# ChenKaiXuSan/Skiing_Analysis_PyTorch

Measured on AMD Instinct MI355X. Metric: 3D-pose frames/sec, 8-view 518px clips, higher is better.
Workload: dtype f16

## Files before the change

skiing_analysis_pytorch_amd/csrc/common.h:

```cpp
#pragma once
#include <hip/hip_runtime.h>
#include <stdint.h>
#include <stdio.h>
#include <atomic>
#include <string>

#include "../../include/skimi.h"

namespace skimi {

void set_error(const char* fmt, ...);

#define SKIMI_CHECK_ARG(cond, ...)            \
    do {                                      \
        if (!(cond)) {                        \
            ::skimi::set_error(__VA_ARGS__);  \
            return SKIMI_ERR_ARG;             \
        }                                     \
    } while (0)

#define SKIMI_HIP(call)                                                                  \
    do {                                                                                 \
        hipError_t e_ = (call);                                                          \
        if (e_ != hipSuccess) {                                                          \
// ... 58 lines not shown
typedef __attribute__((ext_vector_type(8))) _Float16 f16x8;
template <bool F16>
__device__ __forceinline__ f32x16 mfma_32x32x16(bf16x8 a, bf16x8 b, f32x16 c) {
    if constexpr (F16)
        return __builtin_amdgcn_mfma_f32_32x32x16_f16(__builtin_bit_cast(f16x8, a), __builtin_bit_cast(f16x8, b), c, 0, 0, 0);
    else
        return __builtin_amdgcn_mfma_f32_32x32x16_bf16(a, b, c, 0, 0, 0);
}
template <bool F16>
__device__ __forceinline__ f32x4 mfma_16x16x32(bf16x8 a, bf16x8 b, f32x4 c) {
    if constexpr (F16)
        return __builtin_amdgcn_mfma_f32_16x16x32_f16(__builtin_bit_cast(f16x8, a), __builtin_bit_cast(f16x8, b), c, 0, 0, 0);
    else
        return __builtin_amdgcn_mfma_f32_16x16x32_bf16(a, b, c, 0, 0, 0);
}
__device__ __forceinline__ unsigned mx_scale_byte(float amax) {
    if (!(amax > 0.f)) return 0u;
    const float t = amax * (1.0f / 448.0f);
    const unsigned u = __float_as_uint(t);
    const int e = (int)((u >> 23) & 0xFF) - 127 + ((u & 0x7FFFFF) ? 1 : 0);
    return (unsigned)min(max(e + 127, 1), 254);
}
__device__ __forceinline__ float mx_inv_scale(unsigned sb) { return sb ? __uint_as_float((unsigned)(254 - (int)sb) << 23) : 0.f; }
__device__ __forceinline__ int mx_pack4(float a, float b, float c, float d, float inv) {
    int w = 0;
    w = __builtin_amdgcn_cvt_pk_fp8_f32(a * inv, b * inv, w, false);
    w = __builtin_amdgcn_cvt_pk_fp8_f32(c * inv, d * inv, w, true);
    return w;
}
__device__ __forceinline__ float max8(float v) {
// ... 22 lines not shown
```

skiing_analysis_pytorch_amd/csrc/gemm_x3dma.hip:

```cpp
#include <stdlib.h>

#include <algorithm>

#include "common.h"
#include "gemm_epilogue.h"

namespace skimi {

typedef __attribute__((address_space(3))) void lds_void;
typedef __attribute__((address_space(1))) const void gbl_void;

__global__ __launch_bounds__(256) void split_planes_kernel(const float* __restrict__ x, long ld, long rows, int C,
                                                           unsigned short* __restrict__ hi, unsigned short* __restrict__ lo) {
    const int C4 = C / 4;
    const long total = rows * C4;
    for (long i = (long)blockIdx.x * 256 + threadIdx.x; i < total; i += (long)gridDim.x * 256) {
        const long r = i / C4;
        const int c = (int)(i - r * C4) * 4;
        const float4 v = *reinterpret_cast<const float4*>(x + r * ld + c);
        const float f[4] = {v.x, v.y, v.z, v.w};
        bf16x4 h, l;
#pragma unroll
        for (int k = 0; k < 4; ++k) {
            const unsigned short hb = f2bf(f[k]);
// ... 55 lines not shown
    const char* w;
    const char* zero;
    long a_row_bytes;
    long w_row_bytes;
    long a_bias;
};

#define SKIMI_X3_BAR()                        \
    do {                                      \
        __builtin_amdgcn_sched_barrier(0);    \
        __builtin_amdgcn_s_barrier();         \
        __builtin_amdgcn_sched_barrier(0);    \
    } while (0)
#define SKIMI_X3_VMCNT(N) __builtin_amdgcn_s_waitcnt(0x0F70 | ((N) & 15) | (((N) >> 4) << 14))

template <int AMODE, int ABL = 0>
__global__ __launch_bounds__(256, 1) void gemm_x3w4_kernel(const GemmArgs p, const X3Rec pl) {
    constexpr int BM = 256, BN = 256, BK = 32, RB = 128, PIECE = 128 * RB, NSLOT = 10;
    extern __shared__ __attribute__((aligned(16))) char smem[];

    const int tid = threadIdx.x, lane = tid & 63;
    const int wave = __builtin_amdgcn_readfirstlane(tid >> 6);
    const int wr = wave >> 1, wc = wave & 1;
    const int l31 = lane & 31, lh = lane >> 5;

    int id;
    {
        const int nblk = p.ntm * p.ntn;
        const int bid = blockIdx.x;
        const int xcd = bid & 7;
        const int q = nblk >> 3, r = nblk & 7;
        id = (xcd < r ? xcd * (q + 1) : r * (q + 1) + (xcd - r) * q) + (bid >> 3);
// ... 22 lines not shown
                const int rem = m - img * ohw;
                const int oy = rem / p.OW;
                const int iy0 = oy * p.stride - p.pad, ix0 = (rem - oy * p.OW) * p.stride - p.pad;
                a_off[q][j] = (unsigned)((((long)img * p.cH + iy0) * p.cW + ix0) * pl.a_row_bytes + c * 16 + pl.a_bias);
                unsigned ok = 0;
                for (int ky = 0; ky < p.KH; ++ky)
                    for (int kx = 0; kx < p.KW; ++kx) {
                        const int iy = iy0 + ky * p.dil, ix = ix0 + kx * p.dil;
                        if (iy >= 0 && iy < p.cH && ix >= 0 && ix < p.cW) ok |= 1u << (ky * p.KW + kx);
                    }
                a_ok[q][j] = ok;
            }
            w_off[q][j] = (unsigned)((long)min(n0 + 128 * q + row, p.N - 1) * pl.w_row_bytes + c * 16);
        }
    int cur_tap = 0, cur_ky = 0, cur_kx = 0, cur_cs = 0;
    auto issue_a = [&](int kt, int slot0, int slot1) {
        const int tap = cur_tap, tap_dy = cur_ky * p.dil, tap_dx = cur_kx * p.dil;
        const int cs = AMODE == 0 ? kt : cur_cs;
        if (AMODE == 2) {
            ++cur_tap;
            if (++cur_kx == p.KW) { cur_kx = 0; ++cur_ky; }
            if (cur_tap == p.KH * p.KW) { cur_tap = 0; cur_ky = 0; ++cur_cs; }
        } else if (AMODE == 1) {
            if (++cur_cs == p.cC / 32) {
                cur_cs = 0;
                ++cur_tap;
                if (++cur_kx == p.KW) { cur_kx = 0; ++cur_ky; }
            }
        }
        if (ABL & 1) return;
        const long kbytes = ((long)tap_dy * p.cW + tap_dx) * pl.a_row_bytes + (long)cs * 128 - (AMODE != 0 ? pl.a_bias : 0);
        const char* base = pl.a + kbytes;
        const unsigned z = (unsigned)(pl.zero - base);
#pragma unroll
        for (int q = 0; q < 2; ++q) {
            char* dst = smem + (q == 0 ? slot0 : slot1) * PIECE + (4 * wave) * 8 * RB;
#pragma unroll
            for (int j = 0; j < 4; ++j) {
                const bool ok = AMODE == 0 || ((a_ok[q][j] >> tap) & 1u) != 0;
                const unsigned o = ok ? a_off[q][j] : z + ((lane & 7) << 4);
                __builtin_amdgcn_global_load_lds((gbl_void*)(base + (size_t)o), (lds_void*)(dst + j * 8 * RB), 16, 0, 0);
            }
        }
    };
    auto issue_w = [&](int kt, int slot0, int slot1) {
        if (ABL & 1) return;
        const char* base = pl.w + (long)kt * 128;
#pragma unroll
        for (int q = 0; q < 2; ++q) {
            char* dst = smem + (q == 0 ? slot0 : slot1) * PIECE + (4 * wave) * 8 * RB;
#pragma unroll
            for (int j = 0; j < 4; ++j)
                __builtin_amdgcn_global_load_lds((gbl_void*)(base + (size_t)w_off[q][j]), (lds_void*)(dst + j * 8 * RB), 16, 0, 0);
        }
    };
    auto slot = [&](int x) { return x >= NSLOT ? x - NSLOT : x; };

    const int t = lh ^ ((l31 >> 1) & 7);
    const int lane_off = l31 * RB;
    bf16x8 ah0[4], al0[4], wh0[4], wl0[4], ah1[4], al1[4], wh1[4], wl1[4];
    if (ABL & 2) {
#pragma unroll
        for (int i = 0; i < 4; ++i) {
            const bf16x8 c = {(short)lane, 1, 2, 3, 4, 5, 6, 7};
            ah0[i] = al0[i] = wh0[i] = wl0[i] = ah1[i] = al1[i] = wh1[i] = wl1[i] = c;
        }
    }
    auto read = [&](int sb, int s, bf16x8 (&ah)[4], bf16x8 (&al)[4], bf16x8 (&wh)[4], bf16x8 (&wl)[4]) {
        if (ABL & 2) return;
        const int x = ((2 * s) ^ t) << 4;
        const char* pa = smem + slot(sb + wr) * PIECE + lane_off;
        const char* pw = smem + slot(sb + 2 + wc) * PIECE + lane_off;
#pragma unroll
        for (int i = 0; i < 4; ++i) {
            ah[i] = *reinterpret_cast<const bf16x8*>(pa + i * 32 * RB + x);
            al[i] = *reinterpret_cast<const bf16x8*>(pa + i * 32 * RB + (x ^ 64));
        }
#pragma unroll
        for (int i = 0; i < 4; ++i) {
            wh[i] = *reinterpret_cast<const bf16x8*>(pw + i * 32 * RB + x);
            wl[i] = *reinterpret_cast<const bf16x8*>(pw + i * 32 * RB + (x ^ 64));
        }
    };

    f32x16 acc[4][4];
#pragma unroll
    for (int i = 0; i < 4; ++i)
#pragma unroll
        for (int j = 0; j < 4; ++j)
#pragma unroll
            for (int r = 0; r < 16; ++r) acc[i][j][r] = 0.f;
#define SKIMI_X3_MFMA(AH, AL, WH, WL)                                                                             \
    do {                                                                                                           \
        if (ABL & 4) break;                                                                                        \
        _Pragma("unroll") for (int j = 0; j < 4; ++j) _Pragma("unroll") for (int i = 0; i < 4; ++i)                \
            acc[i][j] = __builtin_amdgcn_mfma_f32_32x32x16_bf16(AL[i], WH[j], acc[i][j], 0, 0, 0);                 \
        _Pragma("unroll") for (int j = 0; j < 4; ++j) _Pragma("unroll") for (int i = 0; i < 4; ++i)                \
            acc[i][j] = __builtin_amdgcn_mfma_f32_32x32x16_bf16(AH[i], WL[j], acc[i][j], 0, 0, 0);                 \
        _Pragma("unroll") for (int j = 0; j < 4; ++j) _Pragma("unroll") for (int i = 0; i < 4; ++i)                \
            acc[i][j] = __builtin_amdgcn_mfma_f32_32x32x16_bf16(AH[i], WH[j], acc[i][j], 0, 0, 0);                 \
// ... 49 lines not shown
        SKIMI_X3_MFMA(ah1, al1, wh1, wl1);                                          \
        if (N1) SKIMI_X3_TAIL((N2 ? 8 : 0)); else __builtin_amdgcn_sched_barrier(0); \
        sb = nsb;                                                                   \
    } while (0)
    int kt = 0;
    for (; kt + 2 < nkt; ++kt) SKIMI_X3_KTILE(true, true);
    if (kt + 1 < nkt) {
        SKIMI_X3_KTILE(true, false);
        ++kt;
    }
    SKIMI_X3_KTILE(false, false);
#undef SKIMI_X3_KTILE
#undef SKIMI_X3_TAIL
#undef SKIMI_X3_HEAD
#undef SKIMI_X3_MFMA
    __builtin_amdgcn_s_waitcnt(0xC07F);
    SKIMI_X3_BAR();

    float* stg = reinterpret_cast<float*>(smem) + wave * (32 * 128);
    const int n = n0 + wc * 128 + 4 * (lane & 31);
    const bool relu_ok = (p.act == SKIMI_ACT_NONE || p.act == SKIMI_ACT_RELU) &&
                         (p.post_act == SKIMI_ACT_NONE || p.post_act == SKIMI_ACT_RELU);
    const bool fast = p.vec4 && p.store_mode == 0 && p.out_rpb == 0 && p.out_off == 0 && p.out2 == nullptr &&
                      p.out_dtype == SKIMI_F32 && p.gamma == nullptr && relu_ok && (p.resid != nullptr || p.resid2 == nullptr) &&
                      (p.resid == nullptr || p.resid_dtype == SKIMI_F32) &&
                      m0 + BM <= p.M && n0 + BN <= p.N;
    if (fast) {
        const float lo1 = p.act == SKIMI_ACT_RELU ? 0.f : -__builtin_inff();
        const float lo2 = p.post_act == SKIMI_ACT_RELU ? 0.f : -__builtin_inff();
        float4 bs = make_float4(0.f, 0.f, 0.f, 0.f);
        if (p.bias) bs = *reinterpret_cast<const float4*>(p.bias + n);
        const float* rs = reinterpret_cast<const float*>(p.resid);
        const float* rs2 = reinterpret_cast<const float*>(p.resid2);
        float* out = reinterpret_cast<float*>(p.out);
        const int rpb = p.resid_rpb > 0 ? p.resid_rpb : 0x7fffffff;
        auto res_row = [&](long m) {
            const int b = (int)m / rpb;
            return ((long)b * p.resid_bs + ((int)m - b * rpb) + p.resid_off) * p.ldr;
        };
#define SKIMI_X3_EPI_PASS(HAS_RES, HAS_OUT, HAS_REC)                                                                                 \
    _Pragma("unroll") for (int i = 0; i < 4; ++i) {                                                                \
        _Pragma("unroll") for (int j = 0; j < 4; ++j) _Pragma("unroll") for (int r = 0; r < 16; ++r)               \
            stg[((r & 3) + 8 * (r >> 2) + 4 * lh) * 128 + j * 32 + l31] = acc[i][j][r];                           \
        __builtin_amdgcn_fence(__ATOMIC_RELEASE, "wavefront");                                                     \
        __builtin_amdgcn_s_waitcnt(0xC07F);                                                                        \
        _Pragma("unroll") for (int half = 0; half < 2; ++half) {                                                   \
            const long mrow = m0 + wr * 128 + i * 32 + half * 16 + lh;                                             \
            float4 v[8], rr[8], r2[8];                                                                             \
            _Pragma("unroll") for (int it = 0; it < 8; ++it)                                                       \
                v[it] = *reinterpret_cast<const float4*>(&stg[(half * 16 + it * 2 + lh) * 128 + 4 * (lane & 31)]); \
            if (HAS_RES) _Pragma("unroll") for (int it = 0; it < 8; ++it)                                          \
                rr[it] = *reinterpret_cast<const float4*>(rs + res_row(mrow + it * 2) + n);                       \
            if (HAS_RES == 2) _Pragma("unroll") for (int it = 0; it < 8; ++it)                                     \
                r2[it] = *reinterpret_cast<const float4*>(rs2 + (mrow + it * 2) * p.ldr2 + n);                     \
            _Pragma("unroll") for (int it = 0; it < 8; ++it) {                                                     \
                float4 y = make_float4(fmaxf(v[it].x + bs.x, lo1), fmaxf(v[it].y + bs.y, lo1),                     \
                                       fmaxf(v[it].z + bs.z, lo1), fmaxf(v[it].w + bs.w, lo1));                    \
                if (HAS_RES) { y.x += rr[it].x; y.y += rr[it].y; y.z += rr[it].z; y.w += rr[it].w; }               \
                if (HAS_RES == 2) { y.x += r2[it].x; y.y += r2[it].y; y.z += r2[it].z; y.w += r2[it].w; }          \
                y = make_float4(fmaxf(y.x, lo2), fmaxf(y.y, lo2), fmaxf(y.z, lo2), fmaxf(y.w, lo2));               \
                if (HAS_OUT) *reinterpret_cast<float4*>(out + (mrow + it * 2) * p.ldo + n) = y;                    \
                if (HAS_REC) store_rec4(p, mrow + it * 2, n, y.x, y.y, y.z, y.w);                                  \
            }                                                                                                      \
        }                                                                                                          \
        __builtin_amdgcn_s_waitcnt(0xC07F);                                                                        \
// ... 4 lines not shown
            case 10: SKIMI_X3_EPI_PASS(2, true, false) break;
            case 9: SKIMI_X3_EPI_PASS(2, false, true) break;
            case 7: SKIMI_X3_EPI_PASS(1, true, true) break;
            case 6: SKIMI_X3_EPI_PASS(1, true, false) break;
            case 5: SKIMI_X3_EPI_PASS(1, false, true) break;
            case 3: SKIMI_X3_EPI_PASS(0, true, true) break;
            case 2: SKIMI_X3_EPI_PASS(0, true, false) break;
            case 1: SKIMI_X3_EPI_PASS(0, false, true) break;
            default: break;
        }
#undef SKIMI_X3_EPI_PASS
        return;
    }
#pragma unroll
    for (int i = 0; i < 4; ++i) {
#pragma unroll
        for (int j = 0; j < 4; ++j)
#pragma unroll
            for (int r = 0; r < 16; ++r) stg[((r & 3) + 8 * (r >> 2) + 4 * lh) * 128 + j * 32 + l31] = acc[i][j][r];
        __builtin_amdgcn_fence(__ATOMIC_RELEASE, "wavefront");
        __builtin_amdgcn_s_waitcnt(0xC07F);
#pragma unroll 1
        for (int it = 0; it < 16; ++it) {
            const int row_l = it * 2 + lh;
            const int m = m0 + wr * 128 + i * 32 + row_l;
            if (m >= p.M || n >= p.N) continue;
            const float4 v = *reinterpret_cast<const float4*>(&stg[row_l * 128 + 4 * (lane & 31)]);
            const RowMap rm = row_map(p, m);
            if (p.vec4) {
                store_four(p, rm, n, v);
            } else {
                store_one(p, rm, n, v.x);
                if (n + 1 < p.N) store_one(p, rm, n + 1, v.y);
                if (n + 2 < p.N) store_one(p, rm, n + 2, v.z);
                if (n + 3 < p.N) store_one(p, rm, n + 3, v.w);
            }
        }
        __builtin_amdgcn_s_waitcnt(0xC07F);
    }
}

template <int AMODE>
__global__ __launch_bounds__(256, 1) void gemm_x3w4n_kernel(const GemmArgs p, const X3Rec pl) {
    constexpr int BM = 256, BN = 128, BK = 32, RB = 128, PIECE = 128 * RB, NSLOT = 9;
    extern __shared__ __attribute__((aligned(16))) char smem[];

    const int tid = threadIdx.x, lane = tid & 63;
    const int wave = __builtin_amdgcn_readfirstlane(tid >> 6);
    const int wr = wave >> 1, wc = wave & 1;
    const int l31 = lane & 31, lh = lane >> 5;

    int id;
    {
        const int nblk = p.ntm * p.ntn;
        const int bid = blockIdx.x;
        const int xcd = bid & 7;
        const int q = nblk >> 3, r = nblk & 7;
// ... 24 lines not shown
                const int oy = rem / p.OW;
                const int iy0 = oy * p.stride - p.pad, ix0 = (rem - oy * p.OW) * p.stride - p.pad;
                a_off[q][j] = (unsigned)((((long)img * p.cH + iy0) * p.cW + ix0) * pl.a_row_bytes + c * 16 + pl.a_bias);
                unsigned ok = 0;
                for (int ky = 0; ky < p.KH; ++ky)
                    for (int kx = 0; kx < p.KW; ++kx) {
                        const int iy = iy0 + ky * p.dil, ix = ix0 + kx * p.dil;
                        if (iy >= 0 && iy < p.cH && ix >= 0 && ix < p.cW) ok |= 1u << (ky * p.KW + kx);
                    }
                a_ok[q][j] = ok;
            }
        }
        w_off[j] = (unsigned)((long)min(n0 + row, p.N - 1) * pl.w_row_bytes + c * 16);
    }
    int cur_tap = 0, cur_ky = 0, cur_kx = 0, cur_cs = 0;
    auto issue = [&](int kt, int s0, int s1, int s2) {
        const int tap = cur_tap, tap_dy = cur_ky * p.dil, tap_dx = cur_kx * p.dil;
        const int cs = AMODE == 0 ? kt : cur_cs;
        if (AMODE == 2) {
            ++cur_tap;
            if (++cur_kx == p.KW) { cur_kx = 0; ++cur_ky; }
            if (cur_tap == p.KH * p.KW) { cur_tap = 0; cur_ky = 0; ++cur_cs; }
        } else if (AMODE == 1) {
            if (++cur_cs == p.cC / 32) {
                cur_cs = 0;
                ++cur_tap;
                if (++cur_kx == p.KW) { cur_kx = 0; ++cur_ky; }
            }
        }
        const long kbytes = ((long)tap_dy * p.cW + tap_dx) * pl.a_row_bytes + (long)cs * 128 - (AMODE != 0 ? pl.a_bias : 0);
        const char* base = pl.a + kbytes;
        const unsigned z = (unsigned)(pl.zero - base);
#pragma unroll
        for (int q = 0; q < 2; ++q) {
            char* dst = smem + (q == 0 ? s0 : s1) * PIECE + (4 * wave) * 8 * RB;
#pragma unroll
            for (int j = 0; j < 4; ++j) {
                const bool ok = AMODE == 0 || ((a_ok[q][j] >> tap) & 1u) != 0;
                const unsigned o = ok ? a_off[q][j] : z + ((lane & 7) << 4);
                __builtin_amdgcn_global_load_lds((gbl_void*)(base + (size_t)o), (lds_void*)(dst + j * 8 * RB), 16, 0, 0);
            }
        }
        const char* wbase = pl.w + (long)kt * 128;
        char* dst = smem + s2 * PIECE + (4 * wave) * 8 * RB;
#pragma unroll
        for (int j = 0; j < 4; ++j)
            __builtin_amdgcn_global_load_lds((gbl_void*)(wbase + (size_t)w_off[j]), (lds_void*)(dst + j * 8 * RB), 16, 0, 0);
    };
    auto slot = [&](int x) { return x >= NSLOT ? x - NSLOT : x; };

    const int t = lh ^ ((l31 >> 1) & 7);
    const int fa_off = l31 * RB, fw_off = (wc * 64 + l31) * RB;
    bf16x8 ah0[4], al0[4], wh0[2], wl0[2], ah1[4], al1[4], wh1[2], wl1[2];
    auto read = [&](int sb, int s, bf16x8 (&ah)[4], bf16x8 (&al)[4], bf16x8 (&wh)[2], bf16x8 (&wl)[2]) {
        const int x = ((2 * s) ^ t) << 4;
        const char* pa = smem + slot(sb + wr) * PIECE + fa_off;
        const char* pw = smem + slot(sb + 2) * PIECE + fw_off;
#pragma unroll
        for (int i = 0; i < 4; ++i) {
            ah[i] = *reinterpret_cast<const bf16x8*>(pa + i * 32 * RB + x);
            al[i] = *reinterpret_cast<const bf16x8*>(pa + i * 32 * RB + (x ^ 64));
        }
#pragma unroll
        for (int i = 0; i < 2; ++i) {
            wh[i] = *reinterpret_cast<const bf16x8*>(pw + i * 32 * RB + x);
            wl[i] = *reinterpret_cast<const bf16x8*>(pw + i * 32 * RB + (x ^ 64));
        }
    };

    f32x16 acc[4][2];
#pragma unroll
    for (int i = 0; i < 4; ++i)
#pragma unroll
        for (int j = 0; j < 2; ++j)
#pragma unroll
            for (int r = 0; r < 16; ++r) acc[i][j][r] = 0.f;
#define SKIMI_X3N_MFMA(AH, AL, WH, WL)                                                                            \
    do {                                                                                                           \
        _Pragma("unroll") for (int j = 0; j < 2; ++j) _Pragma("unroll") for (int i = 0; i < 4; ++i)                \
            acc[i][j] = __builtin_amdgcn_mfma_f32_32x32x16_bf16(AL[i], WH[j], acc[i][j], 0, 0, 0);                 \
        _Pragma("unroll") for (int j = 0; j < 2; ++j) _Pragma("unroll") for (int i = 0; i < 4; ++i)                \
            acc[i][j] = __builtin_amdgcn_mfma_f32_32x32x16_bf16(AH[i], WL[j], acc[i][j], 0, 0, 0);                 \
        _Pragma("unroll") for (int j = 0; j < 2; ++j) _Pragma("unroll") for (int i = 0; i < 4; ++i)                \
            acc[i][j] = __builtin_amdgcn_mfma_f32_32x32x16_bf16(AH[i], WH[j], acc[i][j], 0, 0, 0);                 \
    } while (0)
// ... 46 lines not shown
    int kt = 0;
    for (; kt + 3 < nkt; ++kt) SKIMI_X3N_KTILE(true, true, true);
    if (kt + 2 < nkt) {
        SKIMI_X3N_KTILE(true, true, false);
        ++kt;
    }
    if (kt + 1 < nkt) {
        SKIMI_X3N_KTILE(true, false, false);
        ++kt;
    }
    SKIMI_X3N_KTILE(false, false, false);
#undef SKIMI_X3N_KTILE
#undef SKIMI_X3N_TAIL
#undef SKIMI_X3N_HEAD
#undef SKIMI_X3N_MFMA
    __builtin_amdgcn_s_waitcnt(0xC07F);
    SKIMI_X3_BAR();

    float* stg = reinterpret_cast<float*>(smem) + wave * (32 * 64);
    const int n = n0 + wc * 64 + 4 * (lane & 15);
    const bool relu_ok = (p.act == SKIMI_ACT_NONE || p.act == SKIMI_ACT_RELU) &&
                         (p.post_act == SKIMI_ACT_NONE || p.post_act == SKIMI_ACT_RELU);
    const bool fast = p.vec4 && p.store_mode == 0 && p.out_rpb == 0 && p.out_off == 0 && p.out2 == nullptr &&
                      p.out_dtype == SKIMI_F32 && p.gamma == nullptr && relu_ok && (p.resid != nullptr || p.resid2 == nullptr) &&
                      (p.resid == nullptr || p.resid_dtype == SKIMI_F32) &&
                      m0 + BM <= p.M && n0 + BN <= p.N;
    if (fast) {
        const float lo1 = p.act == SKIMI_ACT_RELU ? 0.f : -__builtin_inff();
        const float lo2 = p.post_act == SKIMI_ACT_RELU ? 0.f : -__builtin_inff();
        float4 bs = make_float4(0.f, 0.f, 0.f, 0.f);
        if (p.bias) bs = *reinterpret_cast<const float4*>(p.bias + n);
        const float* rs = reinterpret_cast<const float*>(p.resid);
        const float* rs2 = reinterpret_cast<const float*>(p.resid2);
        float* out = reinterpret_cast<float*>(p.out);
        const int rpb = p.resid_rpb > 0 ? p.resid_rpb : 0x7fffffff;
        auto res_row = [&](long m) {
            const int b = (int)m / rpb;
            return ((long)b * p.resid_bs + ((int)m - b * rpb) + p.resid_off) * p.ldr;
        };
#define SKIMI_X3N_EPI_PASS(HAS_RES, HAS_OUT, HAS_REC)                                                                                \
    _Pragma("unroll") for (int i = 0; i < 4; ++i) {                                                                \
        _Pragma("unroll") for (int j = 0; j < 2; ++j) _Pragma("unroll") for (int r = 0; r < 16; ++r)               \
            stg[((r & 3) + 8 * (r >> 2) + 4 * lh) * 64 + j * 32 + l31] = acc[i][j][r];                            \
        __builtin_amdgcn_fence(__ATOMIC_RELEASE, "wavefront");                                                     \
        __builtin_amdgcn_s_waitcnt(0xC07F);                                                                        \
        const long mrow = m0 + wr * 128 + i * 32 + (lane >> 4);                                                    \
        float4 v[8], rr[8], r2[8];                                                                                 \
        _Pragma("unroll") for (int it = 0; it < 8; ++it)                                                           \
            v[it] = *reinterpret_cast<const float4*>(&stg[(it * 4 + (lane >> 4)) * 64 + 4 * (lane & 15)]);         \
        if (HAS_RES) _Pragma("unroll") for (int it = 0; it < 8; ++it)                                              \
            rr[it] = *reinterpret_cast<const float4*>(rs + res_row(mrow + it * 4) + n);                           \
        if (HAS_RES == 2) _Pragma("unroll") for (int it = 0; it < 8; ++it)                                         \
            r2[it] = *reinterpret_cast<const float4*>(rs2 + (mrow + it * 4) * p.ldr2 + n);                         \
        _Pragma("unroll") for (int it = 0; it < 8; ++it) {                                                         \
            float4 y = make_float4(fmaxf(v[it].x + bs.x, lo1), fmaxf(v[it].y + bs.y, lo1),                         \
                                   fmaxf(v[it].z + bs.z, lo1), fmaxf(v[it].w + bs.w, lo1));                        \
            if (HAS_RES) { y.x += rr[it].x; y.y += rr[it].y; y.z += rr[it].z; y.w += rr[it].w; }                   \
            if (HAS_RES == 2) { y.x += r2[it].x; y.y += r2[it].y; y.z += r2[it].z; y.w += r2[it].w; }              \
            y = make_float4(fmaxf(y.x, lo2), fmaxf(y.y, lo2), fmaxf(y.z, lo2), fmaxf(y.w, lo2));                   \
            if (HAS_OUT) *reinterpret_cast<float4*>(out + (mrow + it * 4) * p.ldo + n) = y;                        \
            if (HAS_REC) store_rec4(p, mrow + it * 4, n, y.x, y.y, y.z, y.w);                                      \
        }                                                                                                          \
        __builtin_amdgcn_s_waitcnt(0xC07F);                                                                        \
    }
// ... 3 lines not shown
            case 10: SKIMI_X3N_EPI_PASS(2, true, false) break;
            case 9: SKIMI_X3N_EPI_PASS(2, false, true) break;
            case 7: SKIMI_X3N_EPI_PASS(1, true, true) break;
            case 6: SKIMI_X3N_EPI_PASS(1, true, false) break;
            case 5: SKIMI_X3N_EPI_PASS(1, false, true) break;
            case 3: SKIMI_X3N_EPI_PASS(0, true, true) break;
            case 2: SKIMI_X3N_EPI_PASS(0, true, false) break;
            case 1: SKIMI_X3N_EPI_PASS(0, false, true) break;
            default: break;
        }
#undef SKIMI_X3N_EPI_PASS
        return;
    }
#pragma unroll
    for (int i = 0; i < 4; ++i) {
#pragma unroll
        for (int j = 0; j < 2; ++j)
#pragma unroll
            for (int r = 0; r < 16; ++r) stg[((r & 3) + 8 * (r >> 2) + 4 * lh) * 64 + j * 32 + l31] = acc[i][j][r];
        __builtin_amdgcn_fence(__ATOMIC_RELEASE, "wavefront");
        __builtin_amdgcn_s_waitcnt(0xC07F);
#pragma unroll 1
        for (int it = 0; it < 8; ++it) {
            const int row_l = it * 4 + (lane >> 4);
            const int m = m0 + wr * 128 + i * 32 + row_l;
            if (m >= p.M || n >= p.N) continue;
            const float4 v = *reinterpret_cast<const float4*>(&stg[row_l * 64 + 4 * (lane & 15)]);
            const RowMap rm = row_map(p, m);
            if (p.vec4) {
                store_four(p, rm, n, v);
            } else {
                store_one(p, rm, n, v.x);
                if (n + 1 < p.N) store_one(p, rm, n + 1, v.y);
                if (n + 2 < p.N) store_one(p, rm, n + 2, v.z);
                if (n + 3 < p.N) store_one(p, rm, n + 3, v.w);
            }
        }
        __builtin_amdgcn_s_waitcnt(0xC07F);
    }
}

static long x3_rows_in(const skimi_gemm_desc* d) { return d->a_mode == 0 ? (long)d->M : (long)d->cN * d->cH * d->cW; }
// ... 17 lines not shown
        return false;
    }
    if (d->store_mode != 0 && d->store_mode != 1) return false;
    if (d->K % 4 != 0) return false;
    if (d->a_mode != 0 && (d->cC % 32 != 0 || d->KH * d->KW > 32)) return false;
    const long kp = ((long)d->K + 31) / 32 * 32;
    const long bias = d->a_mode == 0 ? 0 : ((long)d->pad * d->cW + d->pad) * x3_cp(d) * 4;
    if ((long)gemm_x3dma_scratch_bytes(d) + bias >= (1ll << 32) || (long)d->N * kp * 4 >= (1ll << 32)) return false;
    static const bool dyn = getenv("SKIMI_ENV_DYNAMIC") && atoi(getenv("SKIMI_ENV_DYNAMIC"));
    static long min_tiles = -1;
    if (min_tiles < 0 || dyn) min_tiles = getenv("SKIMI_X3_MIN_TILES") ? atol(getenv("SKIMI_X3_MIN_TILES")) : 160;
    const long tiles = cdiv(d->M, 256) * (d->N > 128 ? cdiv(d->N, 256) : 1);
    return d->M >= (min_tiles <= 1 ? 256 : 4096) && d->N >= 96 && tiles >= min_tiles;
}

template <int AMODE, int ABL = 0>
static int launch_x3w4(GemmArgs& a, const X3Rec& pl, hipStream_t st) {
    constexpr size_t lds = 10ull * 128 * 128;
    SKIMI_LDS_OPT_IN((gemm_x3w4_kernel<AMODE, ABL>), lds, "gemm_x3w4");
    a.ntm = (int)cdiv(a.M, 256);
    a.ntn = (int)cdiv(a.N, 256);
    a.splitk = 1;
    hipLaunchKernelGGL((gemm_x3w4_kernel<AMODE, ABL>), dim3(a.ntm * a.ntn), dim3(256), lds, st, a, pl);
    SKIMI_LAUNCH_CHECK();
    return SKIMI_OK;
}

template <int AMODE>
static int launch_x3w4n(GemmArgs& a, const X3Rec& pl, hipStream_t st) {
    constexpr size_t lds = 9ull * 128 * 128;
    SKIMI_LDS_OPT_IN(gemm_x3w4n_kernel<AMODE>, lds, "gemm_x3w4n");
    a.ntm = (int)cdiv(a.M, 256);
    a.ntn = (int)cdiv(a.N, 128);
    a.splitk = 1;
    hipLaunchKernelGGL(gemm_x3w4n_kernel<AMODE>, dim3(a.ntm * a.ntn), dim3(256), lds, st, a, pl);
    SKIMI_LAUNCH_CHECK();
    return SKIMI_OK;
}

int gemm_x3dma_launch(GemmArgs& a, const skimi_gemm_desc* d, hipStream_t st) {
    const long rows_in = x3_rows_in(d), cp = x3_cp(d);
    const int Cw = d->a_mode == 0 ? d->K : d->cC;
    char* rec = (char*)d->x3_scratch;
    char* zpage = rec + rows_in * cp * 4;
    if (d->a_dtype == SKIMI_BF16X3_REC) {
        rec = (char*)d->A;
        zpage = (char*)d->x3_scratch;
    } else {
        int rc = split_records_launch((const float*)d->A, d->lda, rows_in, Cw, rec, st, zpage);
        if (rc) return rc;
    }
    X3Rec pl;
    pl.a = rec;
    pl.w = (const char*)d->W_split;
    pl.zero = zpage;
    pl.a_row_bytes = cp * 4;
    pl.w_row_bytes = ((long)d->K + 31) / 32 * 32 * 4;
    pl.a_bias = d->a_mode == 0 ? 0 : ((long)d->pad * d->cW + d->pad) * pl.a_row_bytes;
    a.dbg = 0;
    set_gemm_path(d->N <= 128 ? SKIMI_GEMM_PATH_X3DMA_NARROW : SKIMI_GEMM_PATH_X3DMA_WIDE, 0, 0, 0, 1);
    if (d->N <= 128) {
        if (a.a_mode == 0) return launch_x3w4n<0>(a, pl, st);
        if (a.a_mode == 1) return launch_x3w4n<1>(a, pl, st);
        return launch_x3w4n<2>(a, pl, st);
    }
#ifdef SKIMI_ABLATIONS
    if (a.a_mode == 0) {
        static const int abl = getenv("SKIMI_X3_ABL") ? atoi(getenv("SKIMI_X3_ABL")) : 0;
        switch (abl) {
            case 1: return launch_x3w4<0, 1>(a, pl, st);
            case 2: return launch_x3w4<0, 2>(a, pl, st);
            case 3: return launch_x3w4<0, 3>(a, pl, st);
            case 5: return launch_x3w4<0, 5>(a, pl, st);
            case 6: return launch_x3w4<0, 6>(a, pl, st);
            default: break;
        }
    }
    if (a.a_mode == 2) {
        static const int abl = getenv("SKIMI_X3_ABL") ? atoi(getenv("SKIMI_X3_ABL")) : 0;
// ... 17 lines not shown
```

Baseline: 17.35.

## Add 16x16x32 MFMA main loop with interleaved DMA issue to x3 GEMMs

```diff
diff --git a/skiing_analysis_pytorch_amd/csrc/common.h b/skiing_analysis_pytorch_amd/csrc/common.h
--- a/skiing_analysis_pytorch_amd/csrc/common.h
+++ b/skiing_analysis_pytorch_amd/csrc/common.h
@@ -96,6 +96,7 @@
     else
         return __builtin_amdgcn_mfma_f32_16x16x32_bf16(a, b, c, 0, 0, 0);
 }
+__device__ __forceinline__ int slab_at(int r, int c, int W) { return r * W + (c ^ (((r >> 2) & 1) << 4)); }
 __device__ __forceinline__ unsigned mx_scale_byte(float amax) {
     if (!(amax > 0.f)) return 0u;
     const float t = amax * (1.0f / 448.0f);
diff --git a/skiing_analysis_pytorch_amd/csrc/gemm_x3dma.hip b/skiing_analysis_pytorch_amd/csrc/gemm_x3dma.hip
--- a/skiing_analysis_pytorch_amd/csrc/gemm_x3dma.hip
+++ b/skiing_analysis_pytorch_amd/csrc/gemm_x3dma.hip
@@ -93,8 +93,9 @@
     } while (0)
 #define SKIMI_X3_VMCNT(N) __builtin_amdgcn_s_waitcnt(0x0F70 | ((N) & 15) | (((N) >> 4) << 14))
 
-template <int AMODE, int ABL = 0>
+template <int AMODE, int ABL = 0, bool M16 = false>
 __global__ __launch_bounds__(256, 1) void gemm_x3w4_kernel(const GemmArgs p, const X3Rec pl) {
+    static_assert(!(M16 && ABL), "the timing ablations run on the 32x32x16 loop only");
     constexpr int BM = 256, BN = 256, BK = 32, RB = 128, PIECE = 128 * RB, NSLOT = 10;
     extern __shared__ __attribute__((aligned(16))) char smem[];
 
@@ -147,7 +148,8 @@
             w_off[q][j] = (unsigned)((long)min(n0 + 128 * q + row, p.N - 1) * pl.w_row_bytes + c * 16);
         }
     int cur_tap = 0, cur_ky = 0, cur_kx = 0, cur_cs = 0;
-    auto issue_a = [&](int kt, int slot0, int slot1) {
+    struct ABase { const char* base; unsigned z; int tap; };
+    auto a_base = [&](int kt) {
         const int tap = cur_tap, tap_dy = cur_ky * p.dil, tap_dx = cur_kx * p.dil;
         const int cs = AMODE == 0 ? kt : cur_cs;
         if (AMODE == 2) {
@@ -161,18 +163,31 @@
                 if (++cur_kx == p.KW) { cur_kx = 0; ++cur_ky; }
             }
         }
-        if (ABL & 1) return;
         const long kbytes = ((long)tap_dy * p.cW + tap_dx) * pl.a_row_bytes + (long)cs * 128 - (AMODE != 0 ? pl.a_bias : 0);
         const char* base = pl.a + kbytes;
-        const unsigned z = (unsigned)(pl.zero - base);
+        return ABase{base, (unsigned)(pl.zero - base), tap};
+    };
+    auto issue_a_one = [&](const ABase& b, int q, int j, int slot) {
+        const bool ok = AMODE == 0 || ((a_ok[q][j] >> b.tap) & 1u) != 0;
+        const unsigned o = ok ? a_off[q][j] : b.z + ((lane & 7) << 4);
+        __builtin_amdgcn_global_load_lds((gbl_void*)(b.base + (size_t)o), (lds_void*)(smem + slot * PIECE + (4 * wave + j) * 8 * RB),
+                                         16, 0, 0);
+    };
+    auto issue_w_one = [&](int kt, int q, int j, int slot) {
+        __builtin_amdgcn_global_load_lds((gbl_void*)(pl.w + (long)kt * 128 + (size_t)w_off[q][j]),
+                                         (lds_void*)(smem + slot * PIECE + (4 * wave + j) * 8 * RB), 16, 0, 0);
+    };
+    auto issue_a = [&](int kt, int slot0, int slot1) {
+        const ABase b = a_base(kt);
+        if (ABL & 1) return;
 #pragma unroll
         for (int q = 0; q < 2; ++q) {
             char* dst = smem + (q == 0 ? slot0 : slot1) * PIECE + (4 * wave) * 8 * RB;
 #pragma unroll
             for (int j = 0; j < 4; ++j) {
-                const bool ok = AMODE == 0 || ((a_ok[q][j] >> tap) & 1u) != 0;
-                const unsigned o = ok ? a_off[q][j] : z + ((lane & 7) << 4);
-                __builtin_amdgcn_global_load_lds((gbl_void*)(base + (size_t)o), (lds_void*)(dst + j * 8 * RB), 16, 0, 0);
+                const bool ok = AMODE == 0 || ((a_ok[q][j] >> b.tap) & 1u) != 0;
+                const unsigned o = ok ? a_off[q][j] : b.z + ((lane & 7) << 4);
+                __builtin_amdgcn_global_load_lds((gbl_void*)(b.base + (size_t)o), (lds_void*)(dst + j * 8 * RB), 16, 0, 0);
             }
         }
     };
@@ -189,6 +204,104 @@
     };
     auto slot = [&](int x) { return x >= NSLOT ? x - NSLOT : x; };
 
+    f32x16 acc[4][4];
+    f32x4 acc16[8][8];
+    if constexpr (M16) {
+    const int l15 = lane & 15;
+    const int hi_off = l15 * RB + (((lane >> 4) ^ ((l15 >> 1) & 7)) << 4), lo_off = hi_off ^ 64;
+    bf16x8 fal[8], fwh[8], fah[8], fwl[8];
+    auto read_lo_hi = [&](int sb, int g) {
+        if (g < 8) fal[g] = *reinterpret_cast<const bf16x8*>(smem + slot(sb + wr) * PIECE + g * 16 * RB + lo_off);
+        else fwh[g - 8] = *reinterpret_cast<const bf16x8*>(smem + slot(sb + 2 + wc) * PIECE + (g - 8) * 16 * RB + hi_off);
+    };
+    auto read_hi_lo = [&](int sb, int g) {
+        if (g < 8) fah[g] = *reinterpret_cast<const bf16x8*>(smem + slot(sb + wr) * PIECE + g * 16 * RB + hi_off);
+        else fwl[g - 8] = *reinterpret_cast<const bf16x8*>(smem + slot(sb + 2 + wc) * PIECE + (g - 8) * 16 * RB + lo_off);
+    };
+
+#pragma unroll
+    for (int i = 0; i < 8; ++i)
+#pragma unroll
+        for (int j = 0; j < 8; ++j) {
+            acc16[i][j] = f32x4{0.f, 0.f, 0.f, 0.f};
+            asm volatile("" : "+a"(acc16[i][j]));
+        }
+    asm volatile("s_nop 1");
+    auto term = [&](const bf16x8 (&fa)[8], const bf16x8 (&fb)[8], auto&& extra) {
+#pragma unroll
+        for (int j = 0; j < 8; ++j)
+#pragma unroll
+            for (int i = 0; i < 8; ++i) {
+                asm volatile("v_mfma_f32_16x16x32_bf16 %0, %1, %2, %0" : "+a"(acc16[i][j]) : "v"(fa[i]), "v"(fb[j]));
+                extra(8 * j + i);
+                __builtin_amdgcn_sched_barrier(0);
+            }
+    };
+
+    issue_a(0, 0, 1);
+    issue_w(0, 2, 3);
+    if (nkt > 1) {
+        issue_a(1, 4, 5);
+        issue_w(1, 6, 7);
+        SKIMI_X3_VMCNT(16);
+    } else {
+        SKIMI_X3_VMCNT(0);
+    }
+    SKIMI_X3_BAR();
+    int sb = 0;
+#pragma unroll
+    for (int g = 0; g < 16; ++g) read_lo_hi(sb, g);
+#define SKIMI_X3_HEAD()                       \
+    do {                                      \
+        __builtin_amdgcn_s_waitcnt(0xC07F);   \
+        __builtin_amdgcn_sched_barrier(0);    \
+    } while (0)
+#define SKIMI_X3_KTILE(N1, N2)                                                                              \
+    do {                                                                                                    \
+        const int s8 = slot(sb + 8), s9 = slot(sb + 9), s1 = slot(sb + 1), nsb = slot(sb + 4);              \
+        ABase ab{};                                                                                         \
+        if (N2) ab = a_base(kt + 2);                                                                        \
+             \
+        SKIMI_X3_HEAD();                                                                                    \
+        term(fal, fwh, [&](int g) {                                                                         \
+            if (g < 16) read_hi_lo(sb, g);                                                                  \
+            else if (N2 && g < 32 && (g & 1)) {                                                             \
+                const int d = (g - 16) >> 1;                                                                \
+                issue_a_one(ab, d >> 2, d & 3, (d >> 2) ? s9 : s8);                                         \
+            }                                                                                               \
+        });                                                                                                 \
+                                                                                           \
+        SKIMI_X3_HEAD();                                                                                    \
+        term(fah, fwh, [](int) {});                                                                         \
+                                              \
+        if (N1) {                                                                                           \
+            if (N2) SKIMI_X3_VMCNT(8); else SKIMI_X3_VMCNT(0);                                              \
+            SKIMI_X3_BAR();                                                                                 \
+        }                                                                                                   \
+        term(fah, fwl, [&](int g) {                                                                         \
+            if (N1 && g < 16) read_lo_hi(nsb, g);                                                           \
+            else if (N2 && g >= 16 && g < 32 && (g & 1)) {                                                  \
+                const int d = (g - 16) >> 1;                                                                \
+                issue_w_one(kt + 2, d >> 2, d & 3, (d >> 2) ? s1 : sb);                                     \
+            }                                                                                               \
+        });                                                                                                 \
+        sb = nsb;                                                                                           \
+    } while (0)
+    int kt = 0;
+    for (; kt + 2 < nkt; ++kt) SKIMI_X3_KTILE(true, true);
+    if (kt + 1 < nkt) {
+        SKIMI_X3_KTILE(true, false);
+        ++kt;
+    }
+    SKIMI_X3_KTILE(false, false);
+#undef SKIMI_X3_KTILE
+#undef SKIMI_X3_HEAD
+    asm volatile("s_nop 7\n\ts_nop 4");
+#pragma unroll
+    for (int i = 0; i < 8; ++i)
+#pragma unroll
+        for (int j = 0; j < 8; ++j) asm volatile("" : "+a"(acc16[i][j]));
+    } else {
     const int t = lh ^ ((l31 >> 1) & 7);
     const int lane_off = l31 * RB;
     bf16x8 ah0[4], al0[4], wh0[4], wl0[4], ah1[4], al1[4], wh1[4], wl1[4];
@@ -216,7 +329,6 @@
         }
     };
 
-    f32x16 acc[4][4];
 #pragma unroll
     for (int i = 0; i < 4; ++i)
 #pragma unroll
@@ -296,11 +408,30 @@
 #undef SKIMI_X3_TAIL
 #undef SKIMI_X3_HEAD
 #undef SKIMI_X3_MFMA
+    }
     __builtin_amdgcn_s_waitcnt(0xC07F);
     SKIMI_X3_BAR();
 
     float* stg = reinterpret_cast<float*>(smem) + wave * (32 * 128);
     const int n = n0 + wc * 128 + 4 * (lane & 31);
+    const int sw16 = (lane & 16);
+    auto to_slab = [&](int i) {
+        if constexpr (M16) {
+#pragma unroll
+            for (int b = 0; b < 2; ++b)
+#pragma unroll
+                for (int c = 0; c < 8; ++c)
+#pragma unroll
+                    for (int r = 0; r < 4; ++r)
+                        stg[(16 * b + 4 * (lane >> 4) + r) * 128 + 16 * c + (lane & 15) + ((c & 1) ? -sw16 : sw16)] =
+                            acc16[2 * i + b][c][r];
+        } else {
+#pragma unroll
+            for (int j = 0; j < 4; ++j)
+#pragma unroll
+                for (int r = 0; r < 16; ++r) stg[slab_at((r & 3) + 8 * (r >> 2) + 4 * lh, j * 32 + l31, 128)] = acc[i][j][r];
+        }
+    };
     const bool relu_ok = (p.act == SKIMI_ACT_NONE || p.act == SKIMI_ACT_RELU) &&
                          (p.post_act == SKIMI_ACT_NONE || p.post_act == SKIMI_ACT_RELU);
     const bool fast = p.vec4 && p.store_mode == 0 && p.out_rpb == 0 && p.out_off == 0 && p.out2 == nullptr &&
@@ -322,15 +453,14 @@
         };
 #define SKIMI_X3_EPI_PASS(HAS_RES, HAS_OUT, HAS_REC)                                                                                 \
     _Pragma("unroll") for (int i = 0; i < 4; ++i) {                                                                \
-        _Pragma("unroll") for (int j = 0; j < 4; ++j) _Pragma("unroll") for (int r = 0; r < 16; ++r)               \
-            stg[((r & 3) + 8 * (r >> 2) + 4 * lh) * 128 + j * 32 + l31] = acc[i][j][r];                           \
+        to_slab(i);                                                                                                \
         __builtin_amdgcn_fence(__ATOMIC_RELEASE, "wavefront");                                                     \
         __builtin_amdgcn_s_waitcnt(0xC07F);                                                                        \
         _Pragma("unroll") for (int half = 0; half < 2; ++half) {                                                   \
             const long mrow = m0 + wr * 128 + i * 32 + half * 16 + lh;                                             \
             float4 v[8], rr[8], r2[8];                                                                             \
             _Pragma("unroll") for (int it = 0; it < 8; ++it)                                                       \
-                v[it] = *reinterpret_cast<const float4*>(&stg[(half * 16 + it * 2 + lh) * 128 + 4 * (lane & 31)]); \
+                v[it] = *reinterpret_cast<const float4*>(&stg[(half * 16 + it * 2 + lh) * 128 + ((4 * (lane & 31)) ^ ((it & 2) << 3))]); \
             if (HAS_RES) _Pragma("unroll") for (int it = 0; it < 8; ++it)                                          \
                 rr[it] = *reinterpret_cast<const float4*>(rs + res_row(mrow + it * 2) + n);                       \
             if (HAS_RES == 2) _Pragma("unroll") for (int it = 0; it < 8; ++it)                                     \
@@ -365,10 +495,7 @@
     }
 #pragma unroll
     for (int i = 0; i < 4; ++i) {
-#pragma unroll
-        for (int j = 0; j < 4; ++j)
-#pragma unroll
-            for (int r = 0; r < 16; ++r) stg[((r & 3) + 8 * (r >> 2) + 4 * lh) * 128 + j * 32 + l31] = acc[i][j][r];
+        to_slab(i);
         __builtin_amdgcn_fence(__ATOMIC_RELEASE, "wavefront");
         __builtin_amdgcn_s_waitcnt(0xC07F);
 #pragma unroll 1
@@ -376,7 +503,7 @@
             const int row_l = it * 2 + lh;
             const int m = m0 + wr * 128 + i * 32 + row_l;
             if (m >= p.M || n >= p.N) continue;
-            const float4 v = *reinterpret_cast<const float4*>(&stg[row_l * 128 + 4 * (lane & 31)]);
+            const float4 v = *reinterpret_cast<const float4*>(&stg[slab_at(row_l, 4 * (lane & 31), 128)]);
             const RowMap rm = row_map(p, m);
             if (p.vec4) {
                 store_four(p, rm, n, v);
@@ -391,7 +518,7 @@
     }
 }
 
-template <int AMODE>
+template <int AMODE, bool M16 = false>
 __global__ __launch_bounds__(256, 1) void gemm_x3w4n_kernel(const GemmArgs p, const X3Rec pl) {
     constexpr int BM = 256, BN = 128, BK = 32, RB = 128, PIECE = 128 * RB, NSLOT = 9;
     extern __shared__ __attribute__((aligned(16))) char smem[];
@@ -446,7 +573,8 @@
         w_off[j] = (unsigned)((long)min(n0 + row, p.N - 1) * pl.w_row_bytes + c * 16);
     }
     int cur_tap = 0, cur_ky = 0, cur_kx = 0, cur_cs = 0;
-    auto issue = [&](int kt, int s0, int s1, int s2) {
+    struct ABase { const char* base; unsigned z; int tap; };
+    auto a_base = [&](int kt) {
         const int tap = cur_tap, tap_dy = cur_ky * p.dil, tap_dx = cur_kx * p.dil;
         const int cs = AMODE == 0 ? kt : cur_cs;
         if (AMODE == 2) {
@@ -462,25 +590,117 @@
         }
         const long kbytes = ((long)tap_dy * p.cW + tap_dx) * pl.a_row_bytes + (long)cs * 128 - (AMODE != 0 ? pl.a_bias : 0);
         const char* base = pl.a + kbytes;
-        const unsigned z = (unsigned)(pl.zero - base);
-#pragma unroll
-        for (int q = 0; q < 2; ++q) {
-            char* dst = smem + (q == 0 ? s0 : s1) * PIECE + (4 * wave) * 8 * RB;
-#pragma unroll
-            for (int j = 0; j < 4; ++j) {
-                const bool ok = AMODE == 0 || ((a_ok[q][j] >> tap) & 1u) != 0;
-                const unsigned o = ok ? a_off[q][j] : z + ((lane & 7) << 4);
-                __builtin_amdgcn_global_load_lds((gbl_void*)(base + (size_t)o), (lds_void*)(dst + j * 8 * RB), 16, 0, 0);
+        return ABase{base, (unsigned)(pl.zero - base), tap};
+    };
+    auto issue_one = [&](const ABase& b, int kt, int d, int slot) {
+        const int j = d & 3;
+        char* dst = smem + slot * PIECE + (4 * wave + j) * 8 * RB;
+        if (d < 8) {
+            const int q = d >> 2;
+            const bool ok = AMODE == 0 || ((a_ok[q][j] >> b.tap) & 1u) != 0;
+            const unsigned o = ok ? a_off[q][j] : b.z + ((lane & 7) << 4);
+            __builtin_amdgcn_global_load_lds((gbl_void*)(b.base + (size_t)o), (lds_void*)dst, 16, 0, 0);
+        } else {
+            __builtin_amdgcn_global_load_lds((gbl_void*)(pl.w + (long)kt * 128 + (size_t)w_off[j]), (lds_void*)dst, 16, 0, 0);
+        }
+    };
+    auto issue = [&](int kt, int s0, int s1, int s2) {
+        const ABase b = a_base(kt);
+#pragma unroll
+        for (int d = 0; d < 12; ++d) issue_one(b, kt, d, d < 4 ? s0 : d < 8 ? s1 : s2);
+    };
+    auto slot = [&](int x) { return x >= NSLOT ? x - NSLOT : x; };
+
+    f32x16 acc[4][2];
+    f32x4 acc16[8][4];
+    if constexpr (M16) {
+    const int l15 = lane & 15;
+    const int hi_off = l15 * RB + (((lane >> 4) ^ ((l15 >> 1) & 7)) << 4), lo_off = hi_off ^ 64;
+    const int fw16 = wc * 64 * RB;
+    bf16x8 fal[8], fwh[4], fah[8], fwl[4];
+    auto read_lo_hi = [&](int sb, int g) {
+        if (g < 8) fal[g] = *reinterpret_cast<const bf16x8*>(smem + slot(sb + wr) * PIECE + g * 16 * RB + lo_off);
+        else fwh[g - 8] = *reinterpret_cast<const bf16x8*>(smem + slot(sb + 2) * PIECE + fw16 + (g - 8) * 16 * RB + hi_off);
+    };
+    auto read_hi_lo = [&](int sb, int g) {
+        if (g < 8) fah[g] = *reinterpret_cast<const bf16x8*>(smem + slot(sb + wr) * PIECE + g * 16 * RB + hi_off);
+        else fwl[g - 8] = *reinterpret_cast<const bf16x8*>(smem + slot(sb + 2) * PIECE + fw16 + (g - 8) * 16 * RB + lo_off);
+    };
+#pragma unroll
+    for (int i = 0; i < 8; ++i)
+#pragma unroll
+        for (int j = 0; j < 4; ++j) {
+            acc16[i][j] = f32x4{0.f, 0.f, 0.f, 0.f};
+            asm volatile("" : "+a"(acc16[i][j]));
+        }
+    asm volatile("s_nop 1");
+    auto term = [&](const bf16x8 (&fa)[8], const bf16x8 (&fb)[4], auto&& extra) {
+#pragma unroll
+        for (int j = 0; j < 4; ++j)
+#pragma unroll
+            for (int i = 0; i < 8; ++i) {
+                asm volatile("v_mfma_f32_16x16x32_bf16 %0, %1, %2, %0" : "+a"(acc16[i][j]) : "v"(fa[i]), "v"(fb[j]));
+                extra(8 * j + i);
+                __builtin_amdgcn_sched_barrier(0);
             }
-        }
-        const char* wbase = pl.w + (long)kt * 128;
-        char* dst = smem + s2 * PIECE + (4 * wave) * 8 * RB;
-#pragma unroll
-        for (int j = 0; j < 4; ++j)
-            __builtin_amdgcn_global_load_lds((gbl_void*)(wbase + (size_t)w_off[j]), (lds_void*)(dst + j * 8 * RB), 16, 0, 0);
-    };
-    auto slot = [&](int x) { return x >= NSLOT ? x - NSLOT : x; };
-
+    };
+
+    issue(0, 0, 1, 2);
+    if (nkt > 1) issue(1, 3, 4, 5);
+    if (nkt > 2) issue(2, 6, 7, 8);
+    if (nkt > 2) SKIMI_X3_VMCNT(24); else if (nkt > 1) SKIMI_X3_VMCNT(12); else SKIMI_X3_VMCNT(0);
+    SKIMI_X3_BAR();
+    int sb = 0;
+#pragma unroll
+    for (int g = 0; g < 12; ++g) read_lo_hi(sb, g);
+#define SKIMI_X3N_HEAD()                      \
+    do {                                      \
+        __builtin_amdgcn_s_waitcnt(0xC07F);   \
+        __builtin_amdgcn_sched_barrier(0);    \
+    } while (0)
+#define SKIMI_X3N_KTILE(N1, N2, N3)                                                                        \
+    do {                                                                                                    \
+        const int s1 = slot(sb + 1), s2 = slot(sb + 2), nsb = slot(sb + 3);                                 \
+        SKIMI_X3N_HEAD();                                                                                   \
+        term(fal, fwh, [&](int g) {                                                                         \
+            if (g < 12) read_hi_lo(sb, g);                                                                  \
+        });                                                                                                 \
+        SKIMI_X3N_HEAD();                                                                                   \
+        term(fah, fwh, [](int) {});                                                                         \
+        ABase ab{};                                                                                         \
+        if (N3) ab = a_base(kt + 3);                                                                        \
+        if (N1) {                                                                                           \
+            if (N2) SKIMI_X3_VMCNT(12); else SKIMI_X3_VMCNT(0);                                             \
+            SKIMI_X3_BAR();                                                                                 \
+        }                                                                                                   \
+        term(fah, fwl, [&](int g) {                                                                         \
+            if (N1 && g < 12) read_lo_hi(nsb, g);                                                           \
+            else if (N3 && g >= 12 && g < 24) {                                                             \
+                const int d = g - 12;                                                                       \
+                issue_one(ab, kt + 3, d, d < 4 ? sb : d < 8 ? s1 : s2);                                     \
+            }                                                                                               \
+        });                                                                                                 \
+        sb = nsb;                                                                                           \
+    } while (0)
+    int kt = 0;
+    for (; kt + 3 < nkt; ++kt) SKIMI_X3N_KTILE(true, true, true);
+    if (kt + 2 < nkt) {
+        SKIMI_X3N_KTILE(true, true, false);
+        ++kt;
+    }
+    if (kt + 1 < nkt) {
+        SKIMI_X3N_KTILE(true, false, false);
+        ++kt;
+    }
+    SKIMI_X3N_KTILE(false, false, false);
+#undef SKIMI_X3N_KTILE
+#undef SKIMI_X3N_HEAD
+    asm volatile("s_nop 7\n\ts_nop 4");
+#pragma unroll
+    for (int i = 0; i < 8; ++i)
+#pragma unroll
+        for (int j = 0; j < 4; ++j) asm volatile("" : "+a"(acc16[i][j]));
+    } else {
     const int t = lh ^ ((l31 >> 1) & 7);
     const int fa_off = l31 * RB, fw_off = (wc * 64 + l31) * RB;
     bf16x8 ah0[4], al0[4], wh0[2], wl0[2], ah1[4], al1[4], wh1[2], wl1[2];
@@ -500,7 +720,6 @@
         }
     };
 
-    f32x16 acc[4][2];
 #pragma unroll
     for (int i = 0; i < 4; ++i)
 #pragma unroll
@@ -577,11 +796,30 @@
 #undef SKIMI_X3N_TAIL
 #undef SKIMI_X3N_HEAD
 #undef SKIMI_X3N_MFMA
+    }
     __builtin_amdgcn_s_waitcnt(0xC07F);
     SKIMI_X3_BAR();
 
     float* stg = reinterpret_cast<float*>(smem) + wave * (32 * 64);
     const int n = n0 + wc * 64 + 4 * (lane & 15);
+    const int sw16 = (lane & 16);
+    auto to_slab = [&](int i) {
+        if constexpr (M16) {
+#pragma unroll
+            for (int b = 0; b < 2; ++b)
+#pragma unroll
+                for (int c = 0; c < 4; ++c)
+#pragma unroll
+                    for (int r = 0; r < 4; ++r)
+                        stg[(16 * b + 4 * (lane >> 4) + r) * 64 + 16 * c + (lane & 15) + ((c & 1) ? -sw16 : sw16)] =
+                            acc16[2 * i + b][c][r];
+        } else {
+#pragma unroll
+            for (int j = 0; j < 2; ++j)
+#pragma unroll
+                for (int r = 0; r < 16; ++r) stg[slab_at((r & 3) + 8 * (r >> 2) + 4 * lh, j * 32 + l31, 64)] = acc[i][j][r];
+        }
+    };
     const bool relu_ok = (p.act == SKIMI_ACT_NONE || p.act == SKIMI_ACT_RELU) &&
                          (p.post_act == SKIMI_ACT_NONE || p.post_act == SKIMI_ACT_RELU);
     const bool fast = p.vec4 && p.store_mode == 0 && p.out_rpb == 0 && p.out_off == 0 && p.out2 == nullptr &&
@@ -603,14 +841,13 @@
         };
 #define SKIMI_X3N_EPI_PASS(HAS_RES, HAS_OUT, HAS_REC)                                                                                \
     _Pragma("unroll") for (int i = 0; i < 4; ++i) {                                                                \
-        _Pragma("unroll") for (int j = 0; j < 2; ++j) _Pragma("unroll") for (int r = 0; r < 16; ++r)               \
-            stg[((r & 3) + 8 * (r >> 2) + 4 * lh) * 64 + j * 32 + l31] = acc[i][j][r];                            \
+        to_slab(i);                                                                                                \
         __builtin_amdgcn_fence(__ATOMIC_RELEASE, "wavefront");                                                     \
         __builtin_amdgcn_s_waitcnt(0xC07F);                                                                        \
         const long mrow = m0 + wr * 128 + i * 32 + (lane >> 4);                                                    \
         float4 v[8], rr[8], r2[8];                                                                                 \
         _Pragma("unroll") for (int it = 0; it < 8; ++it)                                                           \
-            v[it] = *reinterpret_cast<const float4*>(&stg[(it * 4 + (lane >> 4)) * 64 + 4 * (lane & 15)]);         \
+            v[it] = *reinterpret_cast<const float4*>(&stg[slab_at(it * 4 + (lane >> 4), 4 * (lane & 15), 64)]);         \
         if (HAS_RES) _Pragma("unroll") for (int it = 0; it < 8; ++it)                                              \
             rr[it] = *reinterpret_cast<const float4*>(rs + res_row(mrow + it * 4) + n);                           \
         if (HAS_RES == 2) _Pragma("unroll") for (int it = 0; it < 8; ++it)                                         \
@@ -644,10 +881,7 @@
     }
 #pragma unroll
     for (int i = 0; i < 4; ++i) {
-#pragma unroll
-        for (int j = 0; j < 2; ++j)
-#pragma unroll
-            for (int r = 0; r < 16; ++r) stg[((r & 3) + 8 * (r >> 2) + 4 * lh) * 64 + j * 32 + l31] = acc[i][j][r];
+        to_slab(i);
         __builtin_amdgcn_fence(__ATOMIC_RELEASE, "wavefront");
         __builtin_amdgcn_s_waitcnt(0xC07F);
 #pragma unroll 1
@@ -655,7 +889,7 @@
             const int row_l = it * 4 + (lane >> 4);
             const int m = m0 + wr * 128 + i * 32 + row_l;
             if (m >= p.M || n >= p.N) continue;
-            const float4 v = *reinterpret_cast<const float4*>(&stg[row_l * 64 + 4 * (lane & 15)]);
+            const float4 v = *reinterpret_cast<const float4*>(&stg[slab_at(row_l, 4 * (lane & 15), 64)]);
             const RowMap rm = row_map(p, m);
             if (p.vec4) {
                 store_four(p, rm, n, v);
@@ -703,26 +937,26 @@
     return d->M >= (min_tiles <= 1 ? 256 : 4096) && d->N >= 96 && tiles >= min_tiles;
 }
 
-template <int AMODE, int ABL = 0>
+template <int AMODE, int ABL = 0, bool M16 = false>
 static int launch_x3w4(GemmArgs& a, const X3Rec& pl, hipStream_t st) {
     constexpr size_t lds = 10ull * 128 * 128;
-    SKIMI_LDS_OPT_IN((gemm_x3w4_kernel<AMODE, ABL>), lds, "gemm_x3w4");
+    SKIMI_LDS_OPT_IN((gemm_x3w4_kernel<AMODE, ABL, M16>), lds, "gemm_x3w4");
     a.ntm = (int)cdiv(a.M, 256);
     a.ntn = (int)cdiv(a.N, 256);
     a.splitk = 1;
-    hipLaunchKernelGGL((gemm_x3w4_kernel<AMODE, ABL>), dim3(a.ntm * a.ntn), dim3(256), lds, st, a, pl);
+    hipLaunchKernelGGL((gemm_x3w4_kernel<AMODE, ABL, M16>), dim3(a.ntm * a.ntn), dim3(256), lds, st, a, pl);
     SKIMI_LAUNCH_CHECK();
     return SKIMI_OK;
 }
 
-template <int AMODE>
+template <int AMODE, bool M16>
 static int launch_x3w4n(GemmArgs& a, const X3Rec& pl, hipStream_t st) {
     constexpr size_t lds = 9ull * 128 * 128;
-    SKIMI_LDS_OPT_IN(gemm_x3w4n_kernel<AMODE>, lds, "gemm_x3w4n");
+    SKIMI_LDS_OPT_IN((gemm_x3w4n_kernel<AMODE, M16>), lds, "gemm_x3w4n");
     a.ntm = (int)cdiv(a.M, 256);
     a.ntn = (int)cdiv(a.N, 128);
     a.splitk = 1;
-    hipLaunchKernelGGL(gemm_x3w4n_kernel<AMODE>, dim3(a.ntm * a.ntn), dim3(256), lds, st, a, pl);
+    hipLaunchKernelGGL((gemm_x3w4n_kernel<AMODE, M16>), dim3(a.ntm * a.ntn), dim3(256), lds, st, a, pl);
     SKIMI_LAUNCH_CHECK();
     return SKIMI_OK;
 }
@@ -747,11 +981,25 @@
     pl.w_row_bytes = ((long)d->K + 31) / 32 * 32 * 4;
     pl.a_bias = d->a_mode == 0 ? 0 : ((long)d->pad * d->cW + d->pad) * pl.a_row_bytes;
     a.dbg = 0;
-    set_gemm_path(d->N <= 128 ? SKIMI_GEMM_PATH_X3DMA_NARROW : SKIMI_GEMM_PATH_X3DMA_WIDE, 0, 0, 0, 1);
+    static const bool dyn = getenv("SKIMI_ENV_DYNAMIC") && atoi(getenv("SKIMI_ENV_DYNAMIC"));
+    static int mfma = -1;
+    if (mfma < 0 || dyn) mfma = getenv("SKIMI_X3_MFMA") ? atoi(getenv("SKIMI_X3_MFMA")) : 16;
+    const bool m16 = mfma != 32;
+    set_gemm_path(d->N <= 128 ? SKIMI_GEMM_PATH_X3DMA_NARROW : SKIMI_GEMM_PATH_X3DMA_WIDE, 0, m16 ? 1 : 2, 0, 1);
     if (d->N <= 128) {
-        if (a.a_mode == 0) return launch_x3w4n<0>(a, pl, st);
-        if (a.a_mode == 1) return launch_x3w4n<1>(a, pl, st);
-        return launch_x3w4n<2>(a, pl, st);
+        if (m16) {
+            if (a.a_mode == 0) return launch_x3w4n<0, true>(a, pl, st);
+            if (a.a_mode == 1) return launch_x3w4n<1, true>(a, pl, st);
+            return launch_x3w4n<2, true>(a, pl, st);
+        }
+        if (a.a_mode == 0) return launch_x3w4n<0, false>(a, pl, st);
+        if (a.a_mode == 1) return launch_x3w4n<1, false>(a, pl, st);
+        return launch_x3w4n<2, false>(a, pl, st);
+    }
+    if (m16) {
+        if (a.a_mode == 0) return launch_x3w4<0, 0, true>(a, pl, st);
+        if (a.a_mode == 1) return launch_x3w4<1, 0, true>(a, pl, st);
+        return launch_x3w4<2, 0, true>(a, pl, st);
     }
 #ifdef SKIMI_ABLATIONS
     if (a.a_mode == 0) {
```

Result: faster. 17.53, median of 6 (+1.1%).
